# HuiGuanLab/DL-DKD

Measured on NVIDIA B200. Metric: query-video pairs scored+ranked/sec, higher is better.
Workload: dtype bf16

## Files before the change

### dl-dkd_b200/csrc/dkd_exact_umma.cu

```cuda
#include "dkd_umma.cuh"
#include "dkd_scan.cuh"

namespace dkd {

constexpr int kXRows = 128;
constexpr int kXKB = 32;
constexpr int kXScanWarps = 4;
constexpr int kXStageWarps = 8;
constexpr int kXStagers = 4 * 32;
constexpr int kXMmaWarp = kXScanWarps + kXStageWarps;
constexpr int kXLoadWarp = kXMmaWarp + 1;
constexpr int kXThreads = (kXLoadWarp + 1) * 32;
constexpr int kXMaxAStages = 7;
constexpr int kXBStages = 3;
constexpr uint32_t kXBPlane = 32 * 128;
constexpr int kXTmemCols = 512;
constexpr uint32_t kXRowPitch = 128;
constexpr uint32_t kXSlotBytes = 32 * kXRowPitch;
constexpr uint32_t kXScanScratch = 32 * kXRows * 4;

struct ExactParams {
  const float* q; int M;
  const float* planes; const float* scale;
  int Nv, T, D;
  int b_bufs;
  int R, Npad;
  const uint8_t* mask;
  float* out_max; int32_t* out_arg; int64_t ld_out;
  const int32_t* vid_ptr; const int32_t* vid_cnt; const int32_t* q_list; const int32_t* out_slot;
  unsigned wait_ns;
  int Nv_real, tile_chunks, tiles_per_chunk;
  int64_t list_stride;
  const int32_t* known_key;
  int64_t known_ld;
  const float2* row_ss;
  const float* bias;
  int relu, n_cols;
};
constexpr int kXGroup = 4;
#ifndef DKD_X_LIST_SCAN
#define DKD_X_LIST_SCAN 0
#endif
#ifndef DKD_X_KNOWN
#define DKD_X_KNOWN 1
#endif
#ifndef DKD_X_STREAM_B0
#define DKD_X_STREAM_B0 0
#endif
#ifndef DKD_X_RING0
#define DKD_X_RING0 5
#endif
constexpr bool kXStreamB0 = DKD_X_STREAM_B0 != 0;
constexpr int kXListScan = DKD_X_LIST_SCAN;
constexpr int kXKnown = DKD_X_KNOWN;
constexpr bool kXTwoPhaseList = kXListScan != 0 || kXKnown != 0;

struct __align__(8) ExactCtl {
  uint64_t a_full[kXMaxAStages], a_empty[kXMaxAStages];
  uint64_t b_full[kXBStages], b_empty[kXBStages];
  uint64_t tmem_full[2], tmem_empty[2];
  uint32_t tmem_base;
};

__device__ __forceinline__ void cp_async16(uint32_t dst, const void* src, uint32_t src_bytes) {
  asm volatile("cp.async.cg.shared.global [%0], [%1], 16, %2;" ::"r"(dst), "l"(src), "r"(src_bytes) : "memory");
}
__device__ __forceinline__ void cp_async_commit() { asm volatile("cp.async.commit_group;" ::: "memory"); }
template <int N>
__device__ __forceinline__ void cp_async_wait() { asm volatile("cp.async.wait_group %0;" ::"n"(N) : "memory"); }
__device__ __forceinline__ void bulk_load(void* dst, const void* src, uint32_t bytes, uint64_t* bar) {
  asm volatile("cp.async.bulk.shared::cluster.global.mbarrier::complete_tx::bytes [%0], [%1], %2, [%3];"
               ::"r"(smem_u32(dst)), "l"(src), "r"(bytes), "r"(smem_u32(bar)) : "memory");
}
__device__ __forceinline__ void fence_proxy_async() { asm volatile("fence.proxy.async.shared::cta;" ::: "memory"); }
__device__ __forceinline__ void split_tf32(float x, uint32_t& hi, uint32_t& lo) {
  hi = (__float_as_uint(x) + 0x1000u) & 0xffffe000u;
  lo = __float_as_uint(x - __uint_as_float(hi));
}

__device__ __forceinline__ void tmem_st_16x256b_x4(uint32_t taddr, const uint32_t* r) {
  asm volatile(
      "tcgen05.st.sync.aligned.16x256b.x4.b32 [%0], {%1,%2,%3,%4,%5,%6,%7,%8,%9,%10,%11,%12,%13,%14,%15,%16};"
      ::"r"(taddr), "r"(r[0]), "r"(r[1]), "r"(r[2]), "r"(r[3]), "r"(r[4]), "r"(r[5]), "r"(r[6]), "r"(r[7]),
        "r"(r[8]), "r"(r[9]), "r"(r[10]), "r"(r[11]), "r"(r[12]), "r"(r[13]), "r"(r[14]), "r"(r[15])
      : "memory");
}
__device__ __forceinline__ void tmem_st_wait() { asm volatile("tcgen05.wait::st.sync.aligned;" ::: "memory"); }

__device__ __forceinline__ void umma_tf32_ts(uint32_t tmem_d, uint32_t tmem_a, uint64_t bdesc, uint32_t idesc, uint32_t accum) {
  asm volatile(
      "{\n\t.reg .pred p;\n\t"
      "setp.ne.b32 p, %4, 0;\n\t"
      "tcgen05.mma.cta_group::1.kind::tf32 [%0], [%1], %2, %3, p;\n\t}"
      ::"r"(tmem_d), "r"(tmem_a), "l"(bdesc), "r"(idesc), "r"(accum)
      : "memory");
}
__host__ __device__ __forceinline__ uint32_t make_idesc_tf32(int n, int m) {
  return (1u << 4) | (2u << 7) | (2u << 10) | ((uint32_t)(n >> 3) << 17) | ((uint32_t)(m >> 4) << 24);
}

__device__ __forceinline__ uint32_t sw128_off(int r, int c) {
  return (uint32_t)((r >> 3) * 1024 + (r & 7) * 128 + ((c ^ (r & 7)) << 4));
}

__device__ __forceinline__ void video_range(const ExactParams& p, int n, int& e0, int& count) {
  if (p.vid_ptr) { e0 = p.vid_ptr[n]; count = p.vid_cnt ? p.vid_cnt[n] : p.vid_ptr[n + 1] - e0; }
  else if (p.list_stride > 0) {
    e0 = (int)((int64_t)n * p.list_stride);
    count = p.vid_cnt[n];
    if (count > (int)p.list_stride) count = (int)p.list_stride;
  }
  else { e0 = 0; count = p.M; }
}

__device__ __forceinline__ void item_range(const ExactParams& p, int item, int& group, int& row0, int& count) {
  group = item / p.tile_chunks;
  const int chunk = item - group * p.tile_chunks;
  row0 = chunk * p.tiles_per_chunk * kXRows;
  const int rows = p.tiles_per_chunk * kXRows;
  count = p.M - row0 < rows ? p.M - row0 : rows;
}

__device__ __forceinline__ void item_range_linear(const ExactParams& p, int item, int& wtile, int& row0, int& count) {
  wtile = item % p.Nv_real;
  const int chunk = item / p.Nv_real;
  row0 = chunk * p.tiles_per_chunk * kXRows;
  const int rows = p.tiles_per_chunk * kXRows;
  count = p.M - row0 < rows ? p.M - row0 : rows;
}

template <int kMode, bool kT32, int kXRing>
__global__ void __launch_bounds__(kXThreads, 1)
exact_umma_kernel(const ExactParams p) {
  constexpr int kDW = kMode == 0 ? 32 : 128;
  constexpr int kScaleBufs = kMode == 2 ? kXGroup : 2;
  constexpr int kStageSets = kMode == 2 ? 1 : 2;
  constexpr int kScanGroups = (kMode == 0 && kXTwoPhaseList) ? 1 : 0;
  constexpr bool kResB = kMode == 0 && !kXStreamB0;
  constexpr uint32_t kXACol0 = 2 * kDW;
  constexpr int kXStages = (kXTmemCols - 2 * kDW) / 64;
  extern __shared__ __align__(1024) uint8_t smem_raw_x[];
  __shared__ __align__(16) float s_scale[kScaleBufs][32 * 32];
  uint8_t* smem = reinterpret_cast<uint8_t*>((reinterpret_cast<uintptr_t>(smem_raw_x) + 1023) & ~(uintptr_t)1023);
  const int num_kb = p.D / kXKB;
  const uint32_t b_buf_bytes = kResB ? (uint32_t)num_kb * 2u * kXBPlane : 2u * (uint32_t)p.Npad * 128u;
  uint8_t* sB = smem;
  uint8_t* sS = sB + (size_t)(kResB ? p.b_bufs : kXBStages) * b_buf_bytes;
  float* sD = reinterpret_cast<float*>(sS + (size_t)(4 * kStageSets) * kXRing * kXSlotBytes);
  ExactCtl* ctl = reinterpret_cast<ExactCtl*>(reinterpret_cast<uint8_t*>(sD) + (size_t)kScanGroups * kXScanScratch);
  const int warp = threadIdx.x >> 5, lane = threadIdx.x & 31;
  const uint32_t b_bufs = (uint32_t)p.b_bufs;

  if (threadIdx.x == 0) {
    for (int i = 0; i < kXStages; ++i) { mbar_init(&ctl->a_full[i], kXStagers); mbar_init(&ctl->a_empty[i], 1); }
    for (int i = 0; i < kXBStages; ++i) { mbar_init(&ctl->b_full[i], 1); mbar_init(&ctl->b_empty[i], 1); }
    for (int i = 0; i < 2; ++i) {
      mbar_init(&ctl->tmem_full[i], 1);
      mbar_init(&ctl->tmem_empty[i], kXScanWarps);
    }
    fence_barrier_init();
  }
  if (warp == kXMmaWarp) {
    asm volatile("tcgen05.alloc.cta_group::1.sync.aligned.shared::cta.b32 [%0], %1;" ::"r"(smem_u32(&ctl->tmem_base)), "n"(kXTmemCols));
    asm volatile("tcgen05.relinquish_alloc_permit.cta_group::1.sync.aligned;");
  }
  tc_fence_before();
  __syncthreads();
  tc_fence_after();
  const uint32_t tmem_base = ctl->tmem_base;

  if (warp >= kXScanWarps && warp < kXScanWarps + 4 * kStageSets) {
    const int quarter = warp & 3, par = (warp - kXScanWarps) >> 2;
    const int g = lane >> 2, t = lane & 3;
    const int cl_row = lane >> 3, cl_chunk = lane & 7;
    const uint32_t a_lane = tmem_base + ((uint32_t)(quarter * 32) << 16) + kXACol0;
    const int sw = warp - kXScanWarps;
    const uint32_t ring0 = smem_u32(sS) + (uint32_t)sw * kXRing * kXSlotBytes;
    const uint8_t* ring_ptr = sS + (size_t)sw * kXRing * kXSlotBytes;
    uint32_t it_base = 0;
    for (int n = blockIdx.x; n < p.Nv; n += gridDim.x) {
      int e0, count, row_base = 0;
      if (kMode == 2) { int g_; item_range(p, n, g_, row_base, count); e0 = 0; }
      else if (kMode == 4) { int g_; item_range_linear(p, n, g_, row_base, count); e0 = 0; }
      else video_range(p, n, e0, count);
      if (count <= 0) continue;
      int ss_tile = -1;
      float2 ss[4];
      const int nitems = ((count + kXRows - 1) / kXRows) * num_kb;
      int t_cached = -1;
      const float* src_cached[8];
      uint32_t live_mask = 0;
      int iss_tile = 0, iss_kb = par;
      while (iss_kb >= num_kb) { iss_kb -= num_kb; ++iss_tile; }
      auto issue = [&](int slot) {
        const int tile = iss_tile, kb = iss_kb;
        iss_kb += kStageSets;
        while (iss_kb >= num_kb) { iss_kb -= num_kb; ++iss_tile; }
        if (tile != t_cached) {
          t_cached = tile;
          live_mask = 0;
#pragma unroll
          for (int i = 0; i < 8; ++i) {
            const int r = tile * kXRows + quarter * 32 + 4 * i + cl_row;
            const bool live = r < count;
            const int64_t qrow = live ? (p.q_list ? (int64_t)p.q_list[e0 + r] : (int64_t)(row_base + r)) : 0;
            src_cached[i] = p.q + qrow * p.D + 4 * cl_chunk;
            live_mask |= (live ? 1u : 0u) << i;
          }
        }
        const uint32_t dst = ring0 + (uint32_t)slot * kXSlotBytes + (uint32_t)cl_row * kXRowPitch +
                             (uint32_t)((cl_chunk ^ ((cl_row & 1) << 2)) << 4);
#pragma unroll
        for (int i = 0; i < 8; ++i)
          cp_async16(dst + (uint32_t)(4 * i) * kXRowPitch, src_cached[i] + kb * kXKB, ((live_mask >> i) & 1u) ? 16u : 0u);
      };
      auto store = [&](int j, int slot_i) {
        const uint8_t* slot = ring_ptr + (size_t)slot_i * kXSlotBytes;
        float4 v[8];
#pragma unroll
        for (int hu = 0; hu < 4; ++hu)
#pragma unroll
          for (int c = 0; c < 2; ++c)
            v[2 * hu + c] = *reinterpret_cast<const float4*>(
                slot + (16 * (hu >> 1) + g + 8 * (hu & 1)) * kXRowPitch + (((4 * c + t) ^ ((g & 1) << 2)) << 4));
        if (kMode == 4) {
          if (p.row_ss) {
            const int tile_j = j / num_kb;
            if (tile_j != ss_tile) {
              ss_tile = tile_j;
#pragma unroll
              for (int hu = 0; hu < 4; ++hu) {
                const int r = tile_j * kXRows + quarter * 32 + 16 * (hu >> 1) + g + 8 * (hu & 1);
                ss[hu] = r < count ? __ldg(p.row_ss + row_base + r) : make_float2(0.f, 0.f);
              }
            }
#pragma unroll
            for (int hu = 0; hu < 4; ++hu)
#pragma unroll
              for (int c = 0; c < 2; ++c) {
                float4& x = v[2 * hu + c];
                x.x = fmaf(x.x, ss[hu].x, ss[hu].y); x.y = fmaf(x.y, ss[hu].x, ss[hu].y);
                x.z = fmaf(x.z, ss[hu].x, ss[hu].y); x.w = fmaf(x.w, ss[hu].x, ss[hu].y);
              }
          }
        }
        const uint32_t it = it_base + (uint32_t)j;
        const uint32_t stage = it % (uint32_t)kXStages;
        const uint32_t phase = (it / (uint32_t)kXStages) & 1u;
        mbar_wait_backoff(&ctl->a_empty[stage], phase ^ 1u, 5 * p.wait_ns);
        tc_fence_after();
#pragma unroll
        for (int h = 0; h < 2; ++h) {
          uint32_t rh[16], rl[16];
#pragma unroll
          for (int u = 0; u < 2; ++u)
#pragma unroll
            for (int c = 0; c < 2; ++c) {
              const float4 x = v[2 * (2 * h + u) + c];
              split_tf32(x.x, rh[4 * (2 * c) + 2 * u + 0], rl[4 * (2 * c) + 2 * u + 0]);
              split_tf32(x.y, rh[4 * (2 * c) + 2 * u + 1], rl[4 * (2 * c) + 2 * u + 1]);
              split_tf32(x.z, rh[4 * (2 * c + 1) + 2 * u + 0], rl[4 * (2 * c + 1) + 2 * u + 0]);
              split_tf32(x.w, rh[4 * (2 * c + 1) + 2 * u + 1], rl[4 * (2 * c + 1) + 2 * u + 1]);
            }
          const uint32_t ta = a_lane + ((uint32_t)(16 * h) << 16) + stage * 64u;
          tmem_st_16x256b_x4(ta, rh);
          tmem_st_16x256b_x4(ta + 32u, rl);
        }
        tmem_st_wait();
        tc_fence_before();
        mbar_arrive(&ctl->a_full[stage]);
      };
      const int nmine = (nitems - par + kStageSets - 1) / kStageSets;
#pragma unroll
      for (int m = 0; m < kXRing - 1; ++m) {
        if (m < nmine) issue(m);
        cp_async_commit();
      }
      for (int m = 0; m < nmine; ++m) {
        if (m + kXRing - 1 < nmine) issue((m + kXRing - 1) % kXRing);
        cp_async_commit();
        cp_async_wait<kXRing - 1>();
        __syncwarp();
        store(kStageSets * m + par, m % kXRing);
        __syncwarp();
      }
      cp_async_wait<0>();
      it_base += (uint32_t)nitems;
    }
  } else if (warp == kXLoadWarp) {
    if (lane == 0) {
      uint32_t vi = 0, itb = 0;
      for (int n = blockIdx.x; n < p.Nv; n += gridDim.x) {
        int e0, count;
        if (kMode == 2) {
          int g_, row0_;
          item_range(p, n, g_, row0_, count);
          if (count <= 0) continue;
          const uint8_t* base = reinterpret_cast<const uint8_t*>(p.planes);
          for (int t0 = 0; t0 < count; t0 += kXRows) {
            for (int kb = 0; kb < num_kb; ++kb, ++itb) {
              const uint32_t bs = itb % (uint32_t)kXBStages;
              mbar_wait_backoff(&ctl->b_empty[bs], ((itb / (uint32_t)kXBStages) & 1u) ^ 1u, 5 * p.wait_ns);
              mbar_expect_tx(&ctl->b_full[bs], b_buf_bytes);
              for (int v = 0; v < kXGroup; ++v) {
                const int vid = min(g_ * kXGroup + v, p.Nv_real - 1);
                const uint8_t* src = base + ((size_t)vid * num_kb + kb) * 2 * kXBPlane;
                bulk_load(sB + (size_t)bs * b_buf_bytes + (size_t)v * kXBPlane, src, kXBPlane, &ctl->b_full[bs]);
                bulk_load(sB + (size_t)bs * b_buf_bytes + (size_t)(kXGroup + v) * kXBPlane, src + kXBPlane, kXBPlane,
                          &ctl->b_full[bs]);
              }
            }
          }
          continue;
        }
        int vid = n;
        if (kMode == 4) { int r0_; item_range_linear(p, n, vid, r0_, count); }
        else video_range(p, n, e0, count);
        if (count <= 0) continue;
        if (kResB) {
          const uint32_t bb = vi % b_bufs;
          mbar_wait_backoff(&ctl->b_empty[bb], ((vi / b_bufs) & 1u) ^ 1u, 5 * p.wait_ns);
          ++vi;
          mbar_expect_tx(&ctl->b_full[bb], b_buf_bytes);
          const uint8_t* src = reinterpret_cast<const uint8_t*>(p.planes) + (size_t)n * b_buf_bytes;
          for (int kb = 0; kb < num_kb; ++kb)
            bulk_load(sB + (size_t)bb * b_buf_bytes + (size_t)kb * 2 * kXBPlane, src + (size_t)kb * 2 * kXBPlane,
                      2 * kXBPlane, &ctl->b_full[bb]);
        } else {
          const uint8_t* src = reinterpret_cast<const uint8_t*>(p.planes) + (size_t)vid * num_kb * b_buf_bytes;
          for (int t0 = 0; t0 < count; t0 += kXRows) {
            for (int kb = 0; kb < num_kb; ++kb, ++itb) {
              const uint32_t bs = itb % (uint32_t)kXBStages;
              mbar_wait_backoff(&ctl->b_empty[bs], ((itb / (uint32_t)kXBStages) & 1u) ^ 1u, 5 * p.wait_ns);
              mbar_expect_tx(&ctl->b_full[bs], b_buf_bytes);
              bulk_load(sB + (size_t)bs * b_buf_bytes, src + (size_t)kb * b_buf_bytes, b_buf_bytes, &ctl->b_full[bs]);
            }
          }
        }
      }
    }
  } else if (warp == kXMmaWarp) {
    const int nb = kMode == 0 ? 32 : p.Npad;
    const uint32_t idesc = make_idesc_tf32(nb, kXRows);
    const uint32_t b_plane = (uint32_t)nb * 128u;
    const bool elected = elect_one();
    const uint64_t bdesc0 = make_smem_desc(smem_u32(sB));
    uint32_t it = 0, vi = 0, tc = 0, itb = 0;
    for (int n = blockIdx.x; n < p.Nv; n += gridDim.x) {
      int e0, count;
      if (kMode == 2) { int g_, r_; item_range(p, n, g_, r_, count); e0 = 0; }
      else if (kMode == 4) { int g_, r_; item_range_linear(p, n, g_, r_, count); e0 = 0; }
      else video_range(p, n, e0, count);
      if (count <= 0) continue;
      uint32_t bb = 0;
      if (kResB) {
        bb = vi % b_bufs;
        mbar_wait_backoff(&ctl->b_full[bb], (vi / b_bufs) & 1u, p.wait_ns);
        ++vi;
      }
      for (int t0 = 0; t0 < count; t0 += kXRows, ++tc) {
        const uint32_t buf = tc & 1u;
        mbar_wait_backoff(&ctl->tmem_empty[buf], ((tc >> 1) & 1u) ^ 1u, p.wait_ns);
        tc_fence_after();
        const uint32_t d_tmem = tmem_base + buf * (uint32_t)kDW;
        for (int kb = 0; kb < num_kb; ++kb, ++it) {
          const uint32_t stage = it % (uint32_t)kXStages;
          const uint32_t phase = (it / (uint32_t)kXStages) & 1u;
          uint32_t bs = 0;
          if (!kResB) {
            bs = itb % (uint32_t)kXBStages;
            mbar_wait_backoff(&ctl->b_full[bs], (itb / (uint32_t)kXBStages) & 1u, p.wait_ns);
            ++itb;
          }
          mbar_wait_backoff(&ctl->a_full[stage], phase, p.wait_ns);
          tc_fence_after();
          if (elected) {
            const uint32_t a_hi = tmem_base + kXACol0 + stage * 64u;
            const uint32_t a_lo = a_hi + 32u;
            const uint64_t b_hi = kResB ? bdesc0 + (uint64_t)((bb * b_buf_bytes + (uint32_t)kb * 2u * b_plane) >> 4)
                                             : bdesc0 + (uint64_t)((bs * b_buf_bytes) >> 4);
            const uint64_t b_lo = b_hi + (uint64_t)(b_plane >> 4);
#pragma unroll
            for (int k = 0; k < 4; ++k) {
              umma_tf32_ts(d_tmem, a_lo + 8 * k, b_hi + 2 * k, idesc, (kb | k) ? 1u : 0u);
              umma_tf32_ts(d_tmem, a_hi + 8 * k, b_lo + 2 * k, idesc, 1u);
              umma_tf32_ts(d_tmem, a_hi + 8 * k, b_hi + 2 * k, idesc, 1u);
            }
            umma_commit(&ctl->a_empty[stage]);
            if (!kResB) umma_commit(&ctl->b_empty[bs]);
          }
          __syncwarp();
        }
        if (elected) umma_commit(&ctl->tmem_full[buf]);
        __syncwarp();
      }
      if (kResB) {
        if (elected) umma_commit(&ctl->b_empty[bb]);
        __syncwarp();
      }
    }
  } else if constexpr (kMode == 2) {
    const int T = p.T, P = T * (T + 1) / 2;
    const int quarter = warp & 3;
    const uint32_t part = warp >= 2 * kXScanWarps ? 1u : 0u;
    const int stid = threadIdx.x;
    uint32_t tc = 0;
    for (int n = blockIdx.x; n < p.Nv; n += gridDim.x) {
      int group, row0, count;
      item_range(p, n, group, row0, count);
      if (count <= 0) continue;
      asm volatile("bar.sync 1, %0;" ::"n"(2 * kXScanWarps * 32) : "memory");
      if (part == 0) {
        for (int v = 0; v < kXGroup; ++v) {
          const int vid = min(group * kXGroup + v, p.Nv_real - 1);
          const float* gsc = p.scale + (int64_t)vid * P;
          const int s_ = stid & 31;
          int base = 0;
          for (int w = 1; w <= T; ++w) {
            if ((w & 3) == (stid >> 5) && s_ + w <= T) s_scale[v][(w - 1) * 32 + s_] = __ldg(gsc + base + s_);
            base += T - w + 1;
          }
        }
      }
      asm volatile("bar.sync 1, %0;" ::"n"(2 * kXScanWarps * 32) : "memory");
      for (int t0 = 0; t0 < count; t0 += kXRows, ++tc) {
        const uint32_t buf = tc & 1u;
        if (buf != part) continue;
        mbar_wait(&ctl->tmem_full[buf], (tc >> 1) & 1u);
        tc_fence_after();
        const int r = row0 + t0 + quarter * 32 + lane;
#pragma unroll 1
        for (int v = 0; v < kXGroup; ++v) {
          uint32_t raw[32];
          tmem_ld32_issue(tmem_base + ((uint32_t)(quarter * 32) << 16) + buf * (uint32_t)kDW + (uint32_t)(32 * v), raw);
          tmem_ld_wait();
          if (v == kXGroup - 1) {
            tc_fence_before();
            __syncwarp();
            if (lane == 0) mbar_arrive(&ctl->tmem_empty[buf]);
          }
          const float* sc = s_scale[v];
          float d[32];
#pragma unroll
          for (int i = 0; i < 32; ++i) d[i] = __uint_as_float(raw[i]);
          float bv0;
          int bi0;
          window_scan_v1<kT32>(d, sc, T, bv0, bi0);
          const int vid = group * kXGroup + v;
          if (r < p.M && t0 + quarter * 32 + lane < count && vid < p.Nv_real) {
            const int64_t o = (int64_t)r * p.ld_out + vid;
            p.out_max[o] = bv0;
            if (p.out_arg) p.out_arg[o] = bi0;
          }
        }
      }
    }
  } else if constexpr (kMode == 0) {
    const int T = p.T, P = T * (T + 1) / 2;
    const int quarter = warp;
    const int stid = threadIdx.x;
    uint32_t tc = 0, vi = 0;
    for (int n = blockIdx.x; n < p.Nv; n += gridDim.x) {
      int e0, count;
      video_range(p, n, e0, count);
      if (count <= 0) continue;
      float* sc = s_scale[vi & 1u];
      {
        const float* gsc = p.scale + (int64_t)n * P;
        const int s_ = stid & 31;
        int base = 0;
        for (int w = 1; w <= T; ++w) {
          if ((w & 3) == (stid >> 5) && s_ + w <= T) sc[(w - 1) * 32 + s_] = __ldg(gsc + base + s_);
          base += T - w + 1;
        }
      }
      asm volatile("bar.sync 1, %0;" ::"n"(kXScanWarps * 32) : "memory");
      ++vi;
      for (int t0 = 0; t0 < count; t0 += kXRows, ++tc) {
        const uint32_t buf = tc & 1u;
        mbar_wait(&ctl->tmem_full[buf], (tc >> 1) & 1u);
        tc_fence_after();
        uint32_t raw[32];
        tmem_ld32_issue(tmem_base + ((uint32_t)(quarter * 32) << 16) + buf * (uint32_t)kDW, raw);
        tmem_ld_wait();
        tc_fence_before();
        __syncwarp();
        if (lane == 0) mbar_arrive(&ctl->tmem_empty[buf]);
        float d[32];
#pragma unroll
        for (int i = 0; i < 32; ++i) d[i] = __uint_as_float(raw[i]);
        float bv0;
        int bi0;
        const int r = t0 + quarter * 32 + lane;
        if constexpr (kT32 && kXTwoPhaseList) {
          float* dcol = sD + quarter * 32 + lane;
          if (kXKnown != 0 && p.known_key) {
            const int qi = r < count ? (p.q_list ? p.q_list[e0 + r] : r) : 0;
            const int key = r < count ? __ldg(p.known_key + (int64_t)qi * p.known_ld + n) : 0;
            window_scan_known<kXKnown == 2>(d, sc, dcol, kXRows, key, bv0, bi0);
          } else if (kXListScan != 0) {
            window_scan_v2<kXListScan == 2>(d, sc, dcol, kXRows, bv0, bi0);
          } else {
            window_scan_v1<kT32>(d, sc, T, bv0, bi0);
          }
        } else {
          window_scan_v1<kT32>(d, sc, T, bv0, bi0);
        }
        if (r < count) {
          const int64_t o = p.out_slot ? (int64_t)p.out_slot[e0 + r]
                            : (p.list_stride > 0 ? (int64_t)p.q_list[e0 + r] * p.ld_out + n
                                                 : (p.vid_ptr ? (int64_t)(e0 + r) : (int64_t)r * p.ld_out + n));
          p.out_max[o] = bv0;
          if (p.out_arg) p.out_arg[o] = bi0;
        }
      }
    }
  } else if constexpr (kMode == 4) {
    const int quarter = warp;
    uint32_t tc = 0;
    for (int n = blockIdx.x; n < p.Nv; n += gridDim.x) {
      int wtile, row0, count;
      item_range_linear(p, n, wtile, row0, count);
      if (count <= 0) continue;
      for (int t0 = 0; t0 < count; t0 += kXRows, ++tc) {
        const uint32_t buf = tc & 1u;
        mbar_wait(&ctl->tmem_full[buf], (tc >> 1) & 1u);
        tc_fence_after();
        const int r = t0 + quarter * 32 + lane;
        const bool live = r < count;
        float* orow = p.out_max + (int64_t)(row0 + (live ? r : 0)) * p.ld_out;
#pragma unroll 1
        for (int c0 = 0; c0 < 128; c0 += 32) {
          uint32_t raw[32];
          tmem_ld32_issue(tmem_base + ((uint32_t)(quarter * 32) << 16) + buf * (uint32_t)kDW + (uint32_t)c0, raw);
          tmem_ld_wait();
          if (c0 == 96) {
            tc_fence_before();
            __syncwarp();
            if (lane == 0) mbar_arrive(&ctl->tmem_empty[buf]);
          }
#pragma unroll
          for (int j = 0; j < 32; j += 4) {
            const int col = wtile * 128 + c0 + j;
            if (live && col < p.n_cols) {
              float4 o = make_float4(__uint_as_float(raw[j]), __uint_as_float(raw[j + 1]), __uint_as_float(raw[j + 2]),
                                     __uint_as_float(raw[j + 3]));
              if (p.bias) {
                const float4 b = __ldg(reinterpret_cast<const float4*>(p.bias + col));
                o.x += b.x; o.y += b.y; o.z += b.z; o.w += b.w;
              }
              if (p.relu) { o.x = fmaxf(o.x, 0.f); o.y = fmaxf(o.y, 0.f); o.z = fmaxf(o.z, 0.f); o.w = fmaxf(o.w, 0.f); }
              *reinterpret_cast<float4*>(orow + col) = o;
            }
          }
        }
      }
    }
  } else {
    const int quarter = warp;
    uint32_t tc = 0;
    for (int n = blockIdx.x; n < p.Nv; n += gridDim.x) {
      int e0, count;
      video_range(p, n, e0, count);
      if (count <= 0) continue;
      const uint8_t* mrow = p.mask ? p.mask + (int64_t)n * p.R : nullptr;
      for (int t0 = 0; t0 < count; t0 += kXRows, ++tc) {
        const uint32_t buf = tc & 1u;
        mbar_wait(&ctl->tmem_full[buf], (tc >> 1) & 1u);
        tc_fence_after();
        float bv = -INFINITY;
        int bi = 0;
        for (int c0 = 0; c0 < p.R; c0 += 32) {
          uint32_t raw[32];
          tmem_ld32_issue(tmem_base + ((uint32_t)(quarter * 32) << 16) + buf * (uint32_t)kDW + (uint32_t)c0, raw);
          tmem_ld_wait();
#pragma unroll
          for (int j = 0; j < 32; ++j) {
            const int r = c0 + j;
            if (r < p.R) {
              float v = __uint_as_float(raw[j]);
              if (mrow && __ldg(mrow + r) == 0) v = DKD_MASKED_SCORE;
              if (v > bv) { bv = v; bi = r; }
            }
          }
        }
        tc_fence_before();
        __syncwarp();
        if (lane == 0) mbar_arrive(&ctl->tmem_empty[buf]);
        const int r = t0 + quarter * 32 + lane;
        if (r < count) {
          const int64_t o = p.out_slot ? (int64_t)p.out_slot[e0 + r]
                                       : (p.vid_ptr ? (int64_t)(e0 + r) : (int64_t)r * p.ld_out + n);
          p.out_max[o] = bv;
          if (p.out_arg) p.out_arg[o] = bi;
        }
      }
    }
  }

  tc_fence_before();
  __syncthreads();
  if (warp == kXMmaWarp) {
    tc_fence_after();
    asm volatile("tcgen05.dealloc.cta_group::1.sync.aligned.b32 %0, %1;" ::"r"(tmem_base), "n"(kXTmemCols));
  }
}

__global__ void pack_rows_tf32_kernel(const float* __restrict__ x, int R, int rpad, int D, float* __restrict__ planes,
                                      int64_t total_rows) {
  const int n = blockIdx.x;
  const int num_kb = D / kXKB;
  const uint32_t plane_bytes = (uint32_t)rpad * 128u;
  uint8_t* dst = reinterpret_cast<uint8_t*>(planes) + (size_t)n * num_kb * 2 * plane_bytes;
  for (int i = threadIdx.x; i < num_kb * rpad * 8; i += blockDim.x) {
    const int kb = i / (rpad * 8), rem = i - kb * rpad * 8;
    const int r = rem >> 3, c8 = rem & 7;
    float4 v = make_float4(0.f, 0.f, 0.f, 0.f);
    if (r < R && (int64_t)n * R + r < total_rows) v = *reinterpret_cast<const float4*>(x + ((int64_t)n * R + r) * D + kb * kXKB + c8 * 4);
    uint2 h0, l0, h1, l1;
    split_tf32(v.x, h0.x, l0.x); split_tf32(v.y, h0.y, l0.y); split_tf32(v.z, h1.x, l1.x); split_tf32(v.w, h1.y, l1.y);
    const int cc = c8 >> 2, tt = c8 & 3;
    const int p0 = 16 * cc + 2 * tt;
    uint8_t* row0 = dst + (size_t)(kb * 2) * plane_bytes;
    uint8_t* d0 = row0 + sw128_off(r, p0 >> 2) + (p0 & 3) * 4;
    uint8_t* d1 = row0 + sw128_off(r, (p0 + 8) >> 2) + (p0 & 3) * 4;
    *reinterpret_cast<uint2*>(d0) = h0;
    *reinterpret_cast<uint2*>(d1) = h1;
    *reinterpret_cast<uint2*>(d0 + plane_bytes) = l0;
    *reinterpret_cast<uint2*>(d1 + plane_bytes) = l1;
  }
}

}

using namespace dkd;

static int row_pad(int R, int clip_mode) { return clip_mode ? 32 : ((R + 15) / 16) * 16; }

extern "C" int64_t dkd_clip_planes_bytes(int32_t Nv, int32_t D) {
  if (Nv < 0 || D <= 0 || D % kXKB != 0) return -1;
  return (int64_t)Nv * (D / kXKB) * 2 * kXBPlane;
}
extern "C" int64_t dkd_row_planes_bytes(int32_t Nv, int32_t R, int32_t D) {
  if (Nv < 0 || R <= 0 || R > 128 || D <= 0 || D % kXKB != 0) return -1;
  return (int64_t)Nv * (D / kXKB) * 2 * row_pad(R, 0) * 128;
}

static int pack_rows(const float* x, int32_t Nv, int32_t R, int32_t rpad, int32_t D, float* planes, void* stream) {
  if (!x || !planes || Nv < 0) return DKD_ERR_ARG;
  if (R <= 0 || R > rpad || D <= 0 || D % kXKB != 0 || D > 512) return DKD_ERR_SHAPE;
  if ((reinterpret_cast<uintptr_t>(x) | reinterpret_cast<uintptr_t>(planes)) & 15) return DKD_ERR_ALIGN;
  if (Nv == 0) return DKD_OK;
  pack_rows_tf32_kernel<<<Nv, 256, 0, (cudaStream_t)stream>>>(x, R, rpad, D, planes, (int64_t)Nv * R);
  DKD_LAUNCH_CHECK();
  return DKD_OK;
}
extern "C" int dkd_pack_clips_tf32(const float* clips, int32_t Nv, int32_t T, int32_t D, float* planes, void* stream) {
  if (T > 32) return DKD_ERR_SHAPE;
  return pack_rows(clips, Nv, T, 32, D, planes, stream);
}
extern "C" int dkd_pack_rows_tf32(const float* xn, int32_t Nv, int32_t R, int32_t D, float* planes, void* stream) {
  if (R > 128) return DKD_ERR_SHAPE;
  return pack_rows(xn, Nv, R, row_pad(R, 0), D, planes, stream);
}

static int launch_exact(int mode, ExactParams p, int32_t D, int32_t T, cudaStream_t st) {
  p.wait_ns = 0u;
  int dev = 0, sms = 0, max_smem = 0;
  DKD_CUDA_TRY(cudaGetDevice(&dev));
  DKD_CUDA_TRY(cudaDeviceGetAttribute(&sms, cudaDevAttrMultiProcessorCount, dev));
  DKD_CUDA_TRY(cudaDeviceGetAttribute(&max_smem, cudaDevAttrMaxSharedMemoryPerBlockOptin, dev));
  const int num_kb = D / kXKB;
  const bool stream0 = mode == 0 && kXStreamB0;
  const int ring = stream0 ? DKD_X_RING0 : ((mode == 0 || mode == 2) && D > 448 ? 2 : 3);
  const int ring_warps = mode == 2 ? 4 : kXStageWarps;
  const int scan_groups = (mode == 0 && kXTwoPhaseList) ? 1 : 0;
  const size_t fixed = sizeof(ExactCtl) + 1024 + 128 + 16384  +
                       (size_t)ring_warps * ring * kXSlotBytes + (size_t)scan_groups * kXScanScratch;
  size_t b_total;
  if (mode == 0 && !stream0) {
    const size_t b_buf = (size_t)num_kb * 2 * kXBPlane;
    if ((size_t)max_smem < fixed + b_buf) return DKD_ERR_SHAPE;
    p.b_bufs = ((size_t)max_smem >= fixed + 2 * b_buf) ? 2 : 1;
    b_total = (size_t)p.b_bufs * b_buf;
  } else {
    p.b_bufs = kXBStages;
    b_total = (size_t)kXBStages * 2 * p.Npad * 128;
    if ((size_t)max_smem < fixed + b_total) return DKD_ERR_SHAPE;
  }
  const size_t smem = fixed - 16384 + b_total;
  const int grid = p.Nv < sms ? p.Nv : sms;
  auto launch = [&](auto kern) -> int {
    DKD_CUDA_TRY(cudaFuncSetAttribute(kern, cudaFuncAttributeMaxDynamicSharedMemorySize, (int)smem));
    kern<<<grid, kXThreads, smem, st>>>(p);
    return DKD_OK;
  };
  int rc;
  if (mode == 0 && stream0) {
    rc = (T == 32) ? launch(exact_umma_kernel<0, true, DKD_X_RING0>) : launch(exact_umma_kernel<0, false, DKD_X_RING0>);
  } else if (mode == 0) {
    if (ring == 3) rc = (T == 32) ? launch(exact_umma_kernel<0, true, 3>) : launch(exact_umma_kernel<0, false, 3>);
    else rc = (T == 32) ? launch(exact_umma_kernel<0, true, 2>) : launch(exact_umma_kernel<0, false, 2>);
  } else if (mode == 2) {
    if (ring == 3) rc = (T == 32) ? launch(exact_umma_kernel<2, true, 3>) : launch(exact_umma_kernel<2, false, 3>);
    else rc = (T == 32) ? launch(exact_umma_kernel<2, true, 2>) : launch(exact_umma_kernel<2, false, 2>);
  } else if (mode == 4) {
    rc = launch(exact_umma_kernel<4, true, 3>);
  } else {
    rc = launch(exact_umma_kernel<1, true, 3>);
  }
  if (rc) return rc;
  DKD_LAUNCH_CHECK();
  return DKD_OK;
}

extern "C" int dkd_score_max_exact(const float* qn, int32_t M, const float* row_planes, int32_t Nv, int32_t R,
                                   int32_t D, const uint8_t* mask, float* out_max, int32_t* out_arg,
                                   int64_t ld_out, const int32_t* vid_ptr, const int32_t* q_list, void* stream) {
  if (!qn || !row_planes || !out_max || M < 0 || Nv < 0) return DKD_ERR_ARG;
  if ((vid_ptr == nullptr) != (q_list == nullptr)) return DKD_ERR_ARG;
  if (R <= 0 || R > 128 || D <= 0 || D % kXKB != 0 || D > 512) return DKD_ERR_SHAPE;
  if (!vid_ptr && ld_out < Nv) return DKD_ERR_ARG;
  if ((reinterpret_cast<uintptr_t>(qn) | reinterpret_cast<uintptr_t>(row_planes)) & 15) return DKD_ERR_ALIGN;
  if (M == 0 || Nv == 0) return DKD_OK;
  ExactParams p{};
  p.q = qn; p.M = M; p.planes = row_planes; p.scale = nullptr;
  p.Nv = Nv; p.T = 0; p.D = D; p.R = R; p.Npad = row_pad(R, 0); p.mask = mask;
  p.out_max = out_max; p.out_arg = out_arg; p.ld_out = ld_out;
  p.vid_ptr = vid_ptr; p.vid_cnt = nullptr; p.q_list = q_list; p.out_slot = nullptr;
  return launch_exact(1, p, D, 0, (cudaStream_t)stream);
}

extern "C" int dkd_clip_score_f32(const float* qn, int32_t M, const float* clip_planes, const float* prop_scale,
                                  int32_t Nv, int32_t T, int32_t D, float* out_max, int32_t* out_arg,
                                  int64_t ld_out, const int32_t* vid_ptr, const int32_t* vid_cnt,
                                  const int32_t* q_list, const int32_t* out_slot, const int32_t* known_key,
                                  int64_t known_ld, void* stream) {
  if (!qn || !clip_planes || !prop_scale || !out_max || M < 0 || Nv < 0) return DKD_ERR_ARG;
  if ((vid_ptr == nullptr) != (q_list == nullptr)) return DKD_ERR_ARG;
  if ((out_slot || vid_cnt) && !vid_ptr) return DKD_ERR_ARG;
  if (known_key && (!vid_ptr || known_ld < Nv || T != 32)) return DKD_ERR_ARG;
  if (T <= 0 || T > 32 || D <= 0 || D % kXKB != 0 || D > 512) return DKD_ERR_SHAPE;
  if (!vid_ptr && ld_out < Nv) return DKD_ERR_ARG;
  if ((reinterpret_cast<uintptr_t>(qn) | reinterpret_cast<uintptr_t>(clip_planes) | reinterpret_cast<uintptr_t>(prop_scale)) & 15)
    return DKD_ERR_ALIGN;
  if (M == 0 || Nv == 0) return DKD_OK;
  ExactParams p{};
  p.q = qn; p.M = M; p.planes = clip_planes; p.scale = prop_scale;
  p.Nv = Nv; p.T = T; p.D = D; p.R = T; p.Npad = 32; p.mask = nullptr;
  p.out_max = out_max; p.out_arg = out_arg; p.ld_out = ld_out;
  p.vid_ptr = vid_ptr; p.vid_cnt = vid_cnt; p.q_list = q_list; p.out_slot = out_slot;
  p.known_key = known_key; p.known_ld = known_ld;
  if (!vid_ptr && Nv >= kXGroup) {
    const int groups = (Nv + kXGroup - 1) / kXGroup;
    const int tiles = (M + kXRows - 1) / kXRows;
    int sms = 148, dev = 0;
    if (cudaGetDevice(&dev) == cudaSuccess) cudaDeviceGetAttribute(&sms, cudaDevAttrMultiProcessorCount, dev);
    int chunks = 1;
    while (chunks < tiles && (int64_t)groups * chunks < (int64_t)sms * 12) ++chunks;
    p.tiles_per_chunk = (tiles + chunks - 1) / chunks;
    p.tile_chunks = (tiles + p.tiles_per_chunk - 1) / p.tiles_per_chunk;
    p.Nv_real = Nv;
    p.Nv = groups * p.tile_chunks;
    p.Npad = 128;
    return launch_exact(2, p, D, T, (cudaStream_t)stream);
  }
  return launch_exact(0, p, D, T, (cudaStream_t)stream);
}

extern "C" int64_t dkd_weight_planes_bytes(int32_t N, int32_t K) {
  if (N <= 0 || K <= 0 || K % kXKB != 0) return -1;
  return (int64_t)((N + 127) / 128) * (K / kXKB) * 2 * 128 * 128;
}

extern "C" int dkd_pack_weight_tf32(const float* w, int32_t N, int32_t K, float* planes, void* stream) {
  if (!w || !planes || N <= 0) return DKD_ERR_ARG;
  if (K <= 0 || K % kXKB != 0) return DKD_ERR_SHAPE;
  if ((reinterpret_cast<uintptr_t>(w) | reinterpret_cast<uintptr_t>(planes)) & 15) return DKD_ERR_ALIGN;
  pack_rows_tf32_kernel<<<(N + 127) / 128, 256, 0, (cudaStream_t)stream>>>(w, 128, 128, K, planes, (int64_t)N);
  DKD_LAUNCH_CHECK();
  return DKD_OK;
}

extern "C" int dkd_linear_exact(const float* x, int64_t M, int32_t K, const float* w_planes, int32_t N,
                                const float* bias, int32_t relu, const float* row_scale_shift, float* out,
                                int64_t ld_out, void* stream) {
  if (!x || !w_planes || !out || M < 0 || N <= 0) return DKD_ERR_ARG;
  if (K <= 0 || K % kXKB != 0 || N % 4 != 0 || ld_out < N || ld_out % 4 != 0 || M > 0x7fffff00LL) return DKD_ERR_SHAPE;
  if ((reinterpret_cast<uintptr_t>(x) | reinterpret_cast<uintptr_t>(w_planes) | reinterpret_cast<uintptr_t>(out) |
       reinterpret_cast<uintptr_t>(bias) | reinterpret_cast<uintptr_t>(row_scale_shift)) & 15)
    return DKD_ERR_ALIGN;
  if (M == 0) return DKD_OK;
  ExactParams p{};
  p.q = x; p.M = (int)M; p.planes = w_planes; p.scale = nullptr;
  p.T = 0; p.D = K; p.R = 128; p.Npad = 128; p.mask = nullptr;
  p.out_max = out; p.out_arg = nullptr; p.ld_out = ld_out;
  p.row_ss = reinterpret_cast<const float2*>(row_scale_shift); p.bias = bias; p.relu = relu; p.n_cols = N;
  const int wtiles = (N + 127) / 128;
  const int tiles = (int)((M + kXRows - 1) / kXRows);
  int sms = 148, dev = 0;
  if (cudaGetDevice(&dev) == cudaSuccess) cudaDeviceGetAttribute(&sms, cudaDevAttrMultiProcessorCount, dev);
  int chunks = 1;
  while (chunks < tiles && (int64_t)wtiles * chunks < (int64_t)sms * 6) ++chunks;
  p.tiles_per_chunk = (tiles + chunks - 1) / chunks;
  p.tile_chunks = (tiles + p.tiles_per_chunk - 1) / p.tiles_per_chunk;
  p.Nv_real = wtiles;
  p.Nv = wtiles * p.tile_chunks;
  return launch_exact(4, p, K, 0, (cudaStream_t)stream);
}

extern "C" int dkd_clip_score_list(const float* qn, int32_t M, const float* clip_planes, const float* prop_scale,
                                   int32_t Nv, int32_t T, int32_t D, float* out_max, int32_t* out_arg, int64_t ld_out,
                                   const int32_t* vid_cnt, const int32_t* q_list, int64_t list_stride, void* stream) {
  if (!qn || !clip_planes || !prop_scale || !out_max || !vid_cnt || !q_list || M < 0 || Nv < 0) return DKD_ERR_ARG;
  if (list_stride <= 0 || ld_out < Nv || (int64_t)Nv * list_stride > 0x7fffffffLL) return DKD_ERR_ARG;
  if (T <= 0 || T > 32 || D <= 0 || D % kXKB != 0 || D > 512) return DKD_ERR_SHAPE;
  if ((reinterpret_cast<uintptr_t>(qn) | reinterpret_cast<uintptr_t>(clip_planes) | reinterpret_cast<uintptr_t>(prop_scale)) & 15)
    return DKD_ERR_ALIGN;
  if (M == 0 || Nv == 0) return DKD_OK;
  ExactParams p{};
  p.q = qn; p.M = M; p.planes = clip_planes; p.scale = prop_scale;
  p.Nv = Nv; p.T = T; p.D = D; p.R = T; p.Npad = 32; p.mask = nullptr;
  p.out_max = out_max; p.out_arg = out_arg; p.ld_out = ld_out;
  p.vid_ptr = nullptr; p.vid_cnt = vid_cnt; p.q_list = q_list; p.out_slot = nullptr; p.list_stride = list_stride;
  return launch_exact(0, p, D, T, (cudaStream_t)stream);
}
```

Before: 1.198 billion.

## Stream resident video B planes through a per-k-block slot ring

The resident-B path of the exact UMMA kernel now splits each video's planes into per-k-block slots in a ring of up to 40 slots, sized from the available shared memory. Previously it used one or two whole-video buffers. Each k-block gets its own full/empty barrier, so the MMA warp can start once the first k-block of the next video arrives and each slot is freed after its last tile. This is meant to overlap B loads with compute at finer grain. The change also precomputes swizzled ring addresses and uses explicit ld.shared.v4 loads in the stager warps, fixes the static shared-memory accounting to match the real s_scale size, and adds optional clock-based per-role stall instrumentation behind a macro.

```diff
diff --git a/dl-dkd_b200/csrc/dkd_exact_umma.cu b/dl-dkd_b200/csrc/dkd_exact_umma.cu
--- a/dl-dkd_b200/csrc/dkd_exact_umma.cu
+++ b/dl-dkd_b200/csrc/dkd_exact_umma.cu
@@ -1,5 +1,7 @@
 #include "dkd_umma.cuh"
 #include "dkd_scan.cuh"
+
+#include <algorithm>
 
 namespace dkd {
 
@@ -13,6 +15,7 @@
 constexpr int kXThreads = (kXLoadWarp + 1) * 32;
 constexpr int kXMaxAStages = 7;
 constexpr int kXBStages = 3;
+constexpr int kXBSlotsMax = 40;
 constexpr uint32_t kXBPlane = 32 * 128;
 constexpr int kXTmemCols = 512;
 constexpr uint32_t kXRowPitch = 128;
@@ -55,9 +58,18 @@
 constexpr int kXKnown = DKD_X_KNOWN;
 constexpr bool kXTwoPhaseList = kXListScan != 0 || kXKnown != 0;
 
+#ifdef DKD_X_ROLE_CLOCKS
+enum { kXClkTotal, kXClkDepbar, kXClkAEmpty, kXClkAFull, kXClkBFull, kXClkBEmpty, kXClkTmemFull, kXClkTmemEmpty,
+       kXClkTiles, kXClkSlots };
+__device__ unsigned long long g_x_role_clk[4][kXClkSlots];
+#define X_CLK(slot, ...) do { const long long c0_ = clock64(); __VA_ARGS__; xclk[slot] += clock64() - c0_; } while (0)
+#else
+#define X_CLK(slot, ...) __VA_ARGS__
+#endif
+
 struct __align__(8) ExactCtl {
   uint64_t a_full[kXMaxAStages], a_empty[kXMaxAStages];
-  uint64_t b_full[kXBStages], b_empty[kXBStages];
+  uint64_t b_full[kXBSlotsMax], b_empty[kXBSlotsMax];
   uint64_t tmem_full[2], tmem_empty[2];
   uint32_t tmem_base;
 };
@@ -71,6 +83,11 @@
 __device__ __forceinline__ void bulk_load(void* dst, const void* src, uint32_t bytes, uint64_t* bar) {
   asm volatile("cp.async.bulk.shared::cluster.global.mbarrier::complete_tx::bytes [%0], [%1], %2, [%3];"
                ::"r"(smem_u32(dst)), "l"(src), "r"(bytes), "r"(smem_u32(bar)) : "memory");
+}
+__device__ __forceinline__ float4 lds128(uint32_t addr) {
+  float4 v;
+  asm volatile("ld.shared.v4.f32 {%0, %1, %2, %3}, [%4];" : "=f"(v.x), "=f"(v.y), "=f"(v.z), "=f"(v.w) : "r"(addr) : "memory");
+  return v;
 }
 __device__ __forceinline__ void fence_proxy_async() { asm volatile("fence.proxy.async.shared::cta;" ::: "memory"); }
 __device__ __forceinline__ void split_tf32(float x, uint32_t& hi, uint32_t& lo) {
@@ -143,17 +160,17 @@
   __shared__ __align__(16) float s_scale[kScaleBufs][32 * 32];
   uint8_t* smem = reinterpret_cast<uint8_t*>((reinterpret_cast<uintptr_t>(smem_raw_x) + 1023) & ~(uintptr_t)1023);
   const int num_kb = p.D / kXKB;
-  const uint32_t b_buf_bytes = kResB ? (uint32_t)num_kb * 2u * kXBPlane : 2u * (uint32_t)p.Npad * 128u;
+  const uint32_t b_buf_bytes = kResB ? 2u * kXBPlane : 2u * (uint32_t)p.Npad * 128u;
   uint8_t* sB = smem;
   uint8_t* sS = sB + (size_t)(kResB ? p.b_bufs : kXBStages) * b_buf_bytes;
   float* sD = reinterpret_cast<float*>(sS + (size_t)(4 * kStageSets) * kXRing * kXSlotBytes);
   ExactCtl* ctl = reinterpret_cast<ExactCtl*>(reinterpret_cast<uint8_t*>(sD) + (size_t)kScanGroups * kXScanScratch);
   const int warp = threadIdx.x >> 5, lane = threadIdx.x & 31;
-  const uint32_t b_bufs = (uint32_t)p.b_bufs;
+  const uint32_t b_slots = (uint32_t)p.b_bufs;
 
   if (threadIdx.x == 0) {
     for (int i = 0; i < kXStages; ++i) { mbar_init(&ctl->a_full[i], kXStagers); mbar_init(&ctl->a_empty[i], 1); }
-    for (int i = 0; i < kXBStages; ++i) { mbar_init(&ctl->b_full[i], 1); mbar_init(&ctl->b_empty[i], 1); }
+    for (int i = 0; i < (kResB ? p.b_bufs : kXBStages); ++i) { mbar_init(&ctl->b_full[i], 1); mbar_init(&ctl->b_empty[i], 1); }
     for (int i = 0; i < 2; ++i) {
       mbar_init(&ctl->tmem_full[i], 1);
       mbar_init(&ctl->tmem_empty[i], kXScanWarps);
@@ -168,6 +185,10 @@
   __syncthreads();
   tc_fence_after();
   const uint32_t tmem_base = ctl->tmem_base;
+#ifdef DKD_X_ROLE_CLOCKS
+  long long xclk[kXClkSlots] = {};
+  const long long xclk0 = clock64();
+#endif
 
   if (warp >= kXScanWarps && warp < kXScanWarps + 4 * kStageSets) {
     const int quarter = warp & 3, par = (warp - kXScanWarps) >> 2;
@@ -176,7 +197,9 @@
     const uint32_t a_lane = tmem_base + ((uint32_t)(quarter * 32) << 16) + kXACol0;
     const int sw = warp - kXScanWarps;
     const uint32_t ring0 = smem_u32(sS) + (uint32_t)sw * kXRing * kXSlotBytes;
-    const uint8_t* ring_ptr = sS + (size_t)sw * kXRing * kXSlotBytes;
+    const uint32_t wr0 = ring0 + (uint32_t)cl_row * kXRowPitch + (uint32_t)((cl_chunk ^ ((cl_row & 1) << 2)) << 4);
+    const uint32_t rd0 = ring0 + (uint32_t)g * kXRowPitch + (uint32_t)((t ^ ((g & 1) << 2)) << 4);
+    const uint32_t rd1 = ring0 + (uint32_t)g * kXRowPitch + (uint32_t)(((4 + t) ^ ((g & 1) << 2)) << 4);
     uint32_t it_base = 0;
     for (int n = blockIdx.x; n < p.Nv; n += gridDim.x) {
       int e0, count, row_base = 0;
@@ -208,21 +231,19 @@
             live_mask |= (live ? 1u : 0u) << i;
           }
         }
-        const uint32_t dst = ring0 + (uint32_t)slot * kXSlotBytes + (uint32_t)cl_row * kXRowPitch +
-                             (uint32_t)((cl_chunk ^ ((cl_row & 1) << 2)) << 4);
+        const uint32_t dst = wr0 + (uint32_t)slot * kXSlotBytes;
 #pragma unroll
         for (int i = 0; i < 8; ++i)
           cp_async16(dst + (uint32_t)(4 * i) * kXRowPitch, src_cached[i] + kb * kXKB, ((live_mask >> i) & 1u) ? 16u : 0u);
       };
       auto store = [&](int j, int slot_i) {
-        const uint8_t* slot = ring_ptr + (size_t)slot_i * kXSlotBytes;
+        const uint32_t slot_off = (uint32_t)slot_i * kXSlotBytes;
         float4 v[8];
 #pragma unroll
-        for (int hu = 0; hu < 4; ++hu)
-#pragma unroll
-          for (int c = 0; c < 2; ++c)
-            v[2 * hu + c] = *reinterpret_cast<const float4*>(
-                slot + (16 * (hu >> 1) + g + 8 * (hu & 1)) * kXRowPitch + (((4 * c + t) ^ ((g & 1) << 2)) << 4));
+        for (int hu = 0; hu < 4; ++hu) {
+          v[2 * hu] = lds128(rd0 + slot_off + (uint32_t)(16 * (hu >> 1) + 8 * (hu & 1)) * kXRowPitch);
+          v[2 * hu + 1] = lds128(rd1 + slot_off + (uint32_t)(16 * (hu >> 1) + 8 * (hu & 1)) * kXRowPitch);
+        }
         if (kMode == 4) {
           if (p.row_ss) {
             const int tile_j = j / num_kb;
@@ -247,7 +268,7 @@
         const uint32_t it = it_base + (uint32_t)j;
         const uint32_t stage = it % (uint32_t)kXStages;
         const uint32_t phase = (it / (uint32_t)kXStages) & 1u;
-        mbar_wait_backoff(&ctl->a_empty[stage], phase ^ 1u, 5 * p.wait_ns);
+        X_CLK(kXClkAEmpty, mbar_wait_backoff(&ctl->a_empty[stage], phase ^ 1u, 5 * p.wait_ns));
         tc_fence_after();
 #pragma unroll
         for (int h = 0; h < 2; ++h) {
@@ -279,7 +300,7 @@
       for (int m = 0; m < nmine; ++m) {
         if (m + kXRing - 1 < nmine) issue((m + kXRing - 1) % kXRing);
         cp_async_commit();
-        cp_async_wait<kXRing - 1>();
+        X_CLK(kXClkDepbar, cp_async_wait<kXRing - 1>());
         __syncwarp();
         store(kStageSets * m + par, m % kXRing);
         __syncwarp();
@@ -300,7 +321,7 @@
           for (int t0 = 0; t0 < count; t0 += kXRows) {
             for (int kb = 0; kb < num_kb; ++kb, ++itb) {
               const uint32_t bs = itb % (uint32_t)kXBStages;
-              mbar_wait_backoff(&ctl->b_empty[bs], ((itb / (uint32_t)kXBStages) & 1u) ^ 1u, 5 * p.wait_ns);
+              X_CLK(kXClkBEmpty, mbar_wait_backoff(&ctl->b_empty[bs], ((itb / (uint32_t)kXBStages) & 1u) ^ 1u, 5 * p.wait_ns));
               mbar_expect_tx(&ctl->b_full[bs], b_buf_bytes);
               for (int v = 0; v < kXGroup; ++v) {
                 const int vid = min(g_ * kXGroup + v, p.Nv_real - 1);
@@ -318,20 +339,19 @@
         else video_range(p, n, e0, count);
         if (count <= 0) continue;
         if (kResB) {
-          const uint32_t bb = vi % b_bufs;
-          mbar_wait_backoff(&ctl->b_empty[bb], ((vi / b_bufs) & 1u) ^ 1u, 5 * p.wait_ns);
-          ++vi;
-          mbar_expect_tx(&ctl->b_full[bb], b_buf_bytes);
-          const uint8_t* src = reinterpret_cast<const uint8_t*>(p.planes) + (size_t)n * b_buf_bytes;
-          for (int kb = 0; kb < num_kb; ++kb)
-            bulk_load(sB + (size_t)bb * b_buf_bytes + (size_t)kb * 2 * kXBPlane, src + (size_t)kb * 2 * kXBPlane,
-                      2 * kXBPlane, &ctl->b_full[bb]);
+          const uint8_t* src = reinterpret_cast<const uint8_t*>(p.planes) + (size_t)n * num_kb * b_buf_bytes;
+          for (int kb = 0; kb < num_kb; ++kb, ++vi) {
+            const uint32_t bs = vi % b_slots;
+            X_CLK(kXClkBEmpty, mbar_wait_backoff(&ctl->b_empty[bs], ((vi / b_slots) & 1u) ^ 1u, 5 * p.wait_ns));
+            mbar_expect_tx(&ctl->b_full[bs], b_buf_bytes);
+            bulk_load(sB + (size_t)bs * b_buf_bytes, src + (size_t)kb * b_buf_bytes, b_buf_bytes, &ctl->b_full[bs]);
+          }
         } else {
           const uint8_t* src = reinterpret_cast<const uint8_t*>(p.planes) + (size_t)vid * num_kb * b_buf_bytes;
           for (int t0 = 0; t0 < count; t0 += kXRows) {
             for (int kb = 0; kb < num_kb; ++kb, ++itb) {
               const uint32_t bs = itb % (uint32_t)kXBStages;
-              mbar_wait_backoff(&ctl->b_empty[bs], ((itb / (uint32_t)kXBStages) & 1u) ^ 1u, 5 * p.wait_ns);
+              X_CLK(kXClkBEmpty, mbar_wait_backoff(&ctl->b_empty[bs], ((itb / (uint32_t)kXBStages) & 1u) ^ 1u, 5 * p.wait_ns));
               mbar_expect_tx(&ctl->b_full[bs], b_buf_bytes);
               bulk_load(sB + (size_t)bs * b_buf_bytes, src + (size_t)kb * b_buf_bytes, b_buf_bytes, &ctl->b_full[bs]);
             }
@@ -352,33 +372,31 @@
       else if (kMode == 4) { int g_, r_; item_range_linear(p, n, g_, r_, count); e0 = 0; }
       else video_range(p, n, e0, count);
       if (count <= 0) continue;
-      uint32_t bb = 0;
-      if (kResB) {
-        bb = vi % b_bufs;
-        mbar_wait_backoff(&ctl->b_full[bb], (vi / b_bufs) & 1u, p.wait_ns);
-        ++vi;
-      }
+      const uint32_t vs0 = vi % b_slots;
       for (int t0 = 0; t0 < count; t0 += kXRows, ++tc) {
         const uint32_t buf = tc & 1u;
-        mbar_wait_backoff(&ctl->tmem_empty[buf], ((tc >> 1) & 1u) ^ 1u, p.wait_ns);
+        X_CLK(kXClkTmemEmpty, mbar_wait_backoff(&ctl->tmem_empty[buf], ((tc >> 1) & 1u) ^ 1u, p.wait_ns));
         tc_fence_after();
         const uint32_t d_tmem = tmem_base + buf * (uint32_t)kDW;
         for (int kb = 0; kb < num_kb; ++kb, ++it) {
           const uint32_t stage = it % (uint32_t)kXStages;
           const uint32_t phase = (it / (uint32_t)kXStages) & 1u;
           uint32_t bs = 0;
-          if (!kResB) {
+          if (kResB) {
+            bs = vs0 + (uint32_t)kb;
+            if (bs >= b_slots) bs -= b_slots;
+            if (t0 == 0) X_CLK(kXClkBFull, mbar_wait_backoff(&ctl->b_full[bs], ((vi + (uint32_t)kb) / b_slots) & 1u, p.wait_ns));
+          } else {
             bs = itb % (uint32_t)kXBStages;
-            mbar_wait_backoff(&ctl->b_full[bs], (itb / (uint32_t)kXBStages) & 1u, p.wait_ns);
+            X_CLK(kXClkBFull, mbar_wait_backoff(&ctl->b_full[bs], (itb / (uint32_t)kXBStages) & 1u, p.wait_ns));
             ++itb;
           }
-          mbar_wait_backoff(&ctl->a_full[stage], phase, p.wait_ns);
+          X_CLK(kXClkAFull, mbar_wait_backoff(&ctl->a_full[stage], phase, p.wait_ns));
           tc_fence_after();
           if (elected) {
             const uint32_t a_hi = tmem_base + kXACol0 + stage * 64u;
             const uint32_t a_lo = a_hi + 32u;
-            const uint64_t b_hi = kResB ? bdesc0 + (uint64_t)((bb * b_buf_bytes + (uint32_t)kb * 2u * b_plane) >> 4)
-                                             : bdesc0 + (uint64_t)((bs * b_buf_bytes) >> 4);
+            const uint64_t b_hi = bdesc0 + (uint64_t)((bs * b_buf_bytes) >> 4);
             const uint64_t b_lo = b_hi + (uint64_t)(b_plane >> 4);
 #pragma unroll
             for (int k = 0; k < 4; ++k) {
@@ -387,17 +405,17 @@
               umma_tf32_ts(d_tmem, a_hi + 8 * k, b_hi + 2 * k, idesc, 1u);
             }
             umma_commit(&ctl->a_empty[stage]);
-            if (!kResB) umma_commit(&ctl->b_empty[bs]);
+            if (!kResB || t0 + kXRows >= count) umma_commit(&ctl->b_empty[bs]);
           }
           __syncwarp();
         }
         if (elected) umma_commit(&ctl->tmem_full[buf]);
+#ifdef DKD_X_ROLE_CLOCKS
+        ++xclk[kXClkTiles];
+#endif
         __syncwarp();
       }
-      if (kResB) {
-        if (elected) umma_commit(&ctl->b_empty[bb]);
-        __syncwarp();
-      }
+      if (kResB) vi += (uint32_t)num_kb;
     }
   } else if constexpr (kMode == 2) {
     const int T = p.T, P = T * (T + 1) / 2;
@@ -426,7 +444,7 @@
       for (int t0 = 0; t0 < count; t0 += kXRows, ++tc) {
         const uint32_t buf = tc & 1u;
         if (buf != part) continue;
-        mbar_wait(&ctl->tmem_full[buf], (tc >> 1) & 1u);
+        X_CLK(kXClkTmemFull, mbar_wait(&ctl->tmem_full[buf], (tc >> 1) & 1u));
         tc_fence_after();
         const int r = row0 + t0 + quarter * 32 + lane;
 #pragma unroll 1
@@ -478,7 +496,7 @@
       ++vi;
       for (int t0 = 0; t0 < count; t0 += kXRows, ++tc) {
         const uint32_t buf = tc & 1u;
-        mbar_wait(&ctl->tmem_full[buf], (tc >> 1) & 1u);
+        X_CLK(kXClkTmemFull, mbar_wait(&ctl->tmem_full[buf], (tc >> 1) & 1u));
         tc_fence_after();
         uint32_t raw[32];
         tmem_ld32_issue(tmem_base + ((uint32_t)(quarter * 32) << 16) + buf * (uint32_t)kDW, raw);
@@ -524,7 +542,7 @@
       if (count <= 0) continue;
       for (int t0 = 0; t0 < count; t0 += kXRows, ++tc) {
         const uint32_t buf = tc & 1u;
-        mbar_wait(&ctl->tmem_full[buf], (tc >> 1) & 1u);
+        X_CLK(kXClkTmemFull, mbar_wait(&ctl->tmem_full[buf], (tc >> 1) & 1u));
         tc_fence_after();
         const int r = t0 + quarter * 32 + lane;
         const bool live = r < count;
@@ -566,7 +584,7 @@
       const uint8_t* mrow = p.mask ? p.mask + (int64_t)n * p.R : nullptr;
       for (int t0 = 0; t0 < count; t0 += kXRows, ++tc) {
         const uint32_t buf = tc & 1u;
-        mbar_wait(&ctl->tmem_full[buf], (tc >> 1) & 1u);
+        X_CLK(kXClkTmemFull, mbar_wait(&ctl->tmem_full[buf], (tc >> 1) & 1u));
         tc_fence_after();
         float bv = -INFINITY;
         int bi = 0;
@@ -598,6 +616,14 @@
     }
   }
 
+#ifdef DKD_X_ROLE_CLOCKS
+  xclk[kXClkTotal] = clock64() - xclk0;
+  if (lane == 0) {
+    const int role = warp == kXMmaWarp ? 2 : warp == kXLoadWarp ? 3
+                     : (warp >= kXScanWarps && warp < kXScanWarps + 4 * kStageSets) ? 1 : 0;
+    for (int i = 0; i < kXClkSlots; ++i) atomicAdd(&g_x_role_clk[role][i], (unsigned long long)xclk[i]);
+  }
+#endif
   tc_fence_before();
   __syncthreads();
   if (warp == kXMmaWarp) {
@@ -675,20 +701,21 @@
   const int ring = stream0 ? DKD_X_RING0 : ((mode == 0 || mode == 2) && D > 448 ? 2 : 3);
   const int ring_warps = mode == 2 ? 4 : kXStageWarps;
   const int scan_groups = (mode == 0 && kXTwoPhaseList) ? 1 : 0;
-  const size_t fixed = sizeof(ExactCtl) + 1024 + 128 + 16384  +
+  const size_t static_smem = (size_t)(mode == 2 ? kXGroup : 2) * 32 * 32 * sizeof(float);
+  const size_t fixed = sizeof(ExactCtl) + 1024 + 128 + static_smem +
                        (size_t)ring_warps * ring * kXSlotBytes + (size_t)scan_groups * kXScanScratch;
   size_t b_total;
   if (mode == 0 && !stream0) {
-    const size_t b_buf = (size_t)num_kb * 2 * kXBPlane;
-    if ((size_t)max_smem < fixed + b_buf) return DKD_ERR_SHAPE;
-    p.b_bufs = ((size_t)max_smem >= fixed + 2 * b_buf) ? 2 : 1;
-    b_total = (size_t)p.b_bufs * b_buf;
+    const size_t b_slot = 2 * kXBPlane;
+    if ((size_t)max_smem < fixed + num_kb * b_slot) return DKD_ERR_SHAPE;
+    p.b_bufs = (int)std::min<size_t>(kXBSlotsMax, ((size_t)max_smem - fixed) / b_slot);
+    b_total = (size_t)p.b_bufs * b_slot;
   } else {
     p.b_bufs = kXBStages;
     b_total = (size_t)kXBStages * 2 * p.Npad * 128;
     if ((size_t)max_smem < fixed + b_total) return DKD_ERR_SHAPE;
   }
-  const size_t smem = fixed - 16384 + b_total;
+  const size_t smem = fixed - static_smem + b_total;
   const int grid = p.Nv < sms ? p.Nv : sms;
   auto launch = [&](auto kern) -> int {
     DKD_CUDA_TRY(cudaFuncSetAttribute(kern, cudaFuncAttributeMaxDynamicSharedMemorySize, (int)smem));
@@ -825,3 +852,14 @@
   p.vid_ptr = nullptr; p.vid_cnt = vid_cnt; p.q_list = q_list; p.out_slot = nullptr; p.list_stride = list_stride;
   return launch_exact(0, p, D, T, (cudaStream_t)stream);
 }
+
+#ifdef DKD_X_ROLE_CLOCKS
+extern "C" int dkd_x_role_clocks(unsigned long long* out) {
+  if (!out) return DKD_ERR_ARG;
+  DKD_CUDA_TRY(cudaDeviceSynchronize());
+  DKD_CUDA_TRY(cudaMemcpyFromSymbol(out, g_x_role_clk, sizeof(g_x_role_clk)));
+  static const unsigned long long zero[4 * kXClkSlots] = {};
+  DKD_CUDA_TRY(cudaMemcpyToSymbol(g_x_role_clk, zero, sizeof(zero)));
+  return DKD_OK;
+}
+#endif
```

Result: no change. 1.187 billion, median of 6 (-0.9%).
